# NVlabs/FoundationPose

Measured on AMD Instinct MI355X. Metric: pose-hypotheses/sec (raster+refine+score), 252 hyp x 160x160 @ 640x480 RGB-D, higher is better.
Workload: dtype f16

## Files before the change

### foundationpose_amd/csrc/linear_ln.hip

```cpp
#include <hip/hip_fp16.h>
#include <stdlib.h>
#include <string.h>
#include <type_traits>
#include "igemm_common.h"
#include "rowops_ln.h"

#ifdef FP_PROFILE_BUILD
__device__ unsigned long long ll_dbg[8];
extern "C" int fp_dbg_linear_ln(unsigned long long* out, int reset) {
  if (reset) { unsigned long long z[8] = {0, 0, 0, 0, 0, 0, ~0ull, 0}; return (int)hipMemcpyToSymbol(HIP_SYMBOL(ll_dbg), z, sizeof(z)); }
  return (int)hipMemcpyFromSymbol(out, HIP_SYMBOL(ll_dbg), 8 * sizeof(unsigned long long));
}
#define LL_CLK(t) const unsigned long long t = wall_clock64()
#else
#define LL_CLK(t)
#endif

namespace {

constexpr int LL_BM = 128, LL_BN = 512, LL_K = 512, LL_NW = 8, LL_THREADS = LL_NW * 64, LL_BK = 32;
constexpr int LL_NK = LL_K / LL_BK;
constexpr int LL_KK = LL_BK / 16;
constexpr int LL_TM = LL_BM / 32;
constexpr int LL_ROWB = LL_BK * 2;
constexpr int LL_A_BLOCK = LL_BM * LL_ROWB;
constexpr int LL_E_BYTES = LL_BM * LL_BN * 2;
constexpr int LL_LDS = LL_E_BYTES + LL_BN * 4;
constexpr int LL_ROWS_PER_WAVE = LL_BM / LL_NW, LL_R = 4;
constexpr int LL_LA = 6, LL_LW = 2;
static_assert(LL_NK * LL_A_BLOCK == LL_E_BYTES && LL_LDS <= 160 * 1024, "tile does not fit the 160 KiB LDS");
static_assert(LL_LA > LL_LW && LL_NK > LL_LA, "request order: A block j + LA - LW goes out just before weight fragment j");

struct LinearLnParams {
  const _Float16* X;
  const _Float16* Wp;
  const float* bias;
  const float* x32;
  const _Float16* tok16;
  const float* pe;
  int S;
  const float* gamma;
  const float* beta;
  float eps;
  float* y32;
  _Float16* y16;
  int M;
  int ldx;
  float* part;
  const _Float16* W2p;
  const float* bias2;
  const _Float16* W1p;
  const float* bias1;
};

__global__ __launch_bounds__(256) void k_pack_w512(const _Float16* __restrict__ W, _Float16* __restrict__ out, int K) {
  const int o = blockIdx.x * 256 + threadIdx.x;
  const int lane = o & 63, i = (o >> 6) & 1, rest = o >> 7, nq = K / 16;
  const int q = rest % nq, w = rest / nq;
  if (w >= LL_BN / 64) return;
  const half8 v = *reinterpret_cast<const half8*>(W + (size_t)(64 * w + 32 * i + (lane & 31)) * K + 16 * q + 8 * (lane >> 5));
  *reinterpret_cast<half8*>(out + (size_t)o * 8) = v;
}

__device__ __forceinline__ int ll_swz(int row) { return (row >> 2) & 3; }

__device__ __forceinline__ void ll_dma16(const __amdgpu_buffer_rsrc_t& rs, void* lds, int voff, int soff) {
  __builtin_amdgcn_raw_ptr_buffer_load_lds(rs, (__attribute__((address_space(3))) void*)lds, 16, voff, soff, 0, 0);
}

__device__ __forceinline__ void ll_wait_vm(int n) {
  switch (n) {
    case 0: asm volatile("s_waitcnt vmcnt(0)" ::: "memory"); break;
    case 1: asm volatile("s_waitcnt vmcnt(1)" ::: "memory"); break;
    case 2: asm volatile("s_waitcnt vmcnt(2)" ::: "memory"); break;
    case 4: asm volatile("s_waitcnt vmcnt(4)" ::: "memory"); break;
    case 5: asm volatile("s_waitcnt vmcnt(5)" ::: "memory"); break;
    case 6: asm volatile("s_waitcnt vmcnt(6)" ::: "memory"); break;
    case 8: asm volatile("s_waitcnt vmcnt(8)" ::: "memory"); break;
    case 9: asm volatile("s_waitcnt vmcnt(9)" ::: "memory"); break;
    case 10: asm volatile("s_waitcnt vmcnt(10)" ::: "memory"); break;
    default: asm volatile("s_waitcnt vmcnt(0)" ::: "memory"); break;
  }
}

__device__ __forceinline__ constexpr int ll_after_w(int k1) {
  int n = 0;
  for (int j = k1 + 1; j < LL_NK && j <= k1 - 1 + LL_LW; ++j) n += 4;
  for (int j = k1 + 1; j <= k1 - 1 + LL_LW; ++j) n += (j + LL_LA - LL_LW < LL_NK) ? 1 : 0;
  return n;
}

template <bool MEAN, bool FFN, bool TAIL = false>
__global__ __launch_bounds__(LL_THREADS, 1) void k_rows512(LinearLnParams p) {
  static_assert(!TAIL || (MEAN && FFN), "the tail form ends in the FFN + token-mean form");
  extern __shared__ __attribute__((aligned(16))) unsigned char smem[];
  const int tid = threadIdx.x, lane = tid & 63;
  const int wid = __builtin_amdgcn_readfirstlane(tid >> 6);
  float* bias_lds = reinterpret_cast<float*>(smem + LL_E_BYTES);
  const int m0 = blockIdx.x * LL_BM;
  LL_CLK(t_start);

  if (wid < 2) {
    float* dst = bias_lds + wid * 256;
    if (p.bias) {
      const __amdgpu_buffer_rsrc_t rs = __builtin_amdgcn_make_buffer_rsrc(const_cast<float*>(p.bias), 0, LL_BN * 4, 0x00020000);
      ll_dma16(rs, dst, lane * 16, wid * 1024);
    } else {
      *reinterpret_cast<float4_*>(dst + lane * 4) = float4_{0.f, 0.f, 0.f, 0.f};
    }
  }

  unsigned aoff32;
  {
    const int row = wid * 16 + lane / 4;
    const int c = (lane % 4) ^ ll_swz(row);
    int m = m0 + row;
    m = m < p.M ? m : p.M - 1;
    aoff32 = (unsigned)(((size_t)m * p.ldx + c * 8) * 2);
  }
  const __amdgpu_buffer_rsrc_t rsA = __builtin_amdgcn_make_buffer_rsrc(const_cast<_Float16*>(p.X), 0, 0x7FFFFFFF, 0x00020000);
  auto request_a = [&](int ks) { ll_dma16(rsA, smem + ks * LL_A_BLOCK + wid * 1024, (int)aoff32, ks * (LL_BK * 2)); };
  half8 wr[LL_LW + 1][LL_KK][2];
  auto request_w = [&](const _Float16* wp, int ks, int slot) {
    const _Float16* src = wp + ((size_t)wid * (LL_K / 16) + ks * LL_KK) * 1024 + lane * 8;
#pragma unroll
    for (int kk = 0; kk < LL_KK; ++kk)
#pragma unroll
      for (int i = 0; i < 2; ++i) wr[slot][kk][i] = *reinterpret_cast<const half8*>(src + (kk * 2 + i) * 512);
  };

  float16_ acc[2][LL_TM];
#pragma unroll
  for (int i = 0; i < 2; ++i)
#pragma unroll
    for (int j = 0; j < LL_TM; ++j)
#pragma unroll
      for (int e = 0; e < 16; ++e) acc[i][j][e] = 0.f;

  const int frow = lane & 31, fhalf = lane >> 5;
  const unsigned char* a_ptr[2][LL_KK];
#pragma unroll
  for (int kk = 0; kk < LL_KK; ++kk) {
    a_ptr[0][kk] = smem + frow * LL_ROWB + (((2 * kk + fhalf) ^ ll_swz(frow)) << 4);
    a_ptr[1][kk] = a_ptr[0][kk] + 8 * LL_A_BLOCK;
  }
  half8 fa[2][LL_TM];
  auto read_a = [&](int ks, int kk, int slot) {
#pragma unroll
    for (int t = 0; t < LL_TM; ++t)
      fa[slot][t] = *reinterpret_cast<const half8*>(a_ptr[ks >> 3][kk] + (ks & 7) * LL_A_BLOCK + t * 32 * LL_ROWB);
  };
  auto mfma_group = [&](int wslot, int kk, int aslot) {
#pragma unroll
    for (int i = 0; i < 2; ++i)
#pragma unroll
      for (int j = 0; j < LL_TM; ++j)
        acc[i][j] = __builtin_amdgcn_mfma_f32_32x32x16_f16(wr[wslot][kk][i], fa[aslot][j], acc[i][j], 0, 0, 0);
  };

#pragma unroll
  for (int j = 0; j < LL_LA - LL_LW; ++j) request_a(j);
#pragma unroll
  for (int j = 0; j < LL_LW; ++j) { request_a(j + LL_LA - LL_LW); request_w(p.Wp, j, j); }
  ll_wait_vm(ll_after_w(0));
  __builtin_amdgcn_s_barrier();
  read_a(0, 0, 0);
#pragma unroll
  for (int ks = 0; ks < LL_NK; ++ks) {
    if (ks + LL_LA < LL_NK) request_a(ks + LL_LA);
    if (ks + LL_LW < LL_NK) request_w(p.Wp, ks + LL_LW, (ks + LL_LW) % (LL_LW + 1));
    read_a(ks, 1, 1);
    __builtin_amdgcn_sched_barrier(0);
    mfma_group(ks % (LL_LW + 1), 0, 0);
    __builtin_amdgcn_sched_barrier(0);
    if (ks + 1 < LL_NK) {
      ll_wait_vm(ll_after_w(ks + 1));
      __builtin_amdgcn_s_barrier();
      read_a(ks + 1, 0, 0);
    }
    __builtin_amdgcn_sched_barrier(0);
    mfma_group(ks % (LL_LW + 1), 1, 1);
    __builtin_amdgcn_sched_barrier(0);
  }
  __syncthreads();
  LL_CLK(t_loop1);
  half8 tk[LL_R];
  float rs[LL_R][8];
  auto tile_row = [&](int k) { return MEAN ? wid * LL_ROWS_PER_WAVE + k : wid + LL_NW * k; };
  auto request_resid = [&](int t0, const float* x32) {
#pragma unroll
    for (int u = 0; u < LL_R; ++u) {
      const int m = m0 + tile_row(t0 + u);
      const int mc = m < p.M ? m : p.M - 1;
      if (x32) {
        load8f(x32 + (size_t)mc * 512 + lane * 8, rs[u]);
      } else {
        tk[u] = *reinterpret_cast<const half8*>(p.tok16 + (size_t)mc * 512 + lane * 8);
        load8f(p.pe + (size_t)((unsigned)mc % (unsigned)p.S) * 512 + lane * 8, rs[u]);
      }
    }
  };
  constexpr bool EARLY_RESID = !FFN;
  const float* const resid32 = TAIL ? p.y32 : p.x32;
  if constexpr (EARLY_RESID) request_resid(0, resid32);

  unsigned char* E = smem;
  LL_CLK(t_pre);
  unsigned erow_off = (unsigned)(frow * (2 * LL_BN));
  int esw = frow & 15, efh = fhalf;
  auto read_e = [&](int q, int slot) {
    const unsigned char* erow = E + erow_off;
#pragma unroll
    for (int j = 0; j < LL_TM; ++j)
      fa[slot][j] = *reinterpret_cast<const half8*>(erow + j * 32 * (2 * LL_BN) + (((2 * q + efh) ^ esw) << 4));
  };
  auto zero_acc = [&]() {
#pragma unroll
    for (int i = 0; i < 2; ++i)
#pragma unroll
      for (int j = 0; j < LL_TM; ++j)
#pragma unroll
        for (int e = 0; e < 16; ++e) acc[i][j][e] = 0.f;
  };
  auto product_from_e = [&](const _Float16* wp) {
    asm volatile("" : "+v"(erow_off), "+v"(esw), "+v"(efh));
#pragma unroll
    for (int j = 0; j < LL_LW; ++j) request_w(wp, j, j);
    read_e(0, 0);
#pragma unroll
    for (int ks = 0; ks < LL_NK; ++ks) {
      if (ks + LL_LW < LL_NK) request_w(wp, ks + LL_LW, (ks + LL_LW) % (LL_LW + 1));
      read_e(2 * ks + 1, 1);
      __builtin_amdgcn_sched_barrier(0);
      mfma_group(ks % (LL_LW + 1), 0, 0);
      __builtin_amdgcn_sched_barrier(0);
      if (ks + 1 < LL_NK) read_e(2 * ks + 2, 0);
      __builtin_amdgcn_sched_barrier(0);
      mfma_group(ks % (LL_LW + 1), 1, 1);
      __builtin_amdgcn_sched_barrier(0);
    }
  };
  auto park = [&](auto relu_c) {
    constexpr bool RELU = decltype(relu_c)::value;
    int lane_p = lane;
    asm volatile("" : "+v"(lane_p));
#pragma unroll
    for (int i = 0; i < 2; ++i) {
#pragma unroll
      for (int g = 0; g < 4; ++g) {
        const int nl = wid * 64 + i * 32 + 8 * g + 4 * (lane_p >> 5);
        const float4_ bv = *reinterpret_cast<const float4_*>(bias_lds + nl);
#pragma unroll
        for (int j = 0; j < LL_TM; ++j) {
          const int ml = j * 32 + (lane_p & 31);
          half4 v;
#pragma unroll
          for (int e = 0; e < 4; ++e) v[e] = (_Float16)(acc[i][j][g * 4 + e] + bv[e]);
          if constexpr (RELU) v = __builtin_elementwise_max(v, half4{0, 0, 0, 0});
          const int chunk = (nl >> 3) ^ (ml & 15);
          *reinterpret_cast<half4*>(E + ml * (2 * LL_BN) + (chunk << 4) + ((nl & 4) << 1)) = v;
        }
      }
    }
  };
  auto load_bias = [&](const float* b) {
    if (wid < 2) {
      float* dst = bias_lds + wid * 256;
      if (b) {
        const __amdgpu_buffer_rsrc_t rs_ = __builtin_amdgcn_make_buffer_rsrc(const_cast<float*>(b), 0, LL_BN * 4, 0x00020000);
        ll_dma16(rs_, dst, lane * 16, wid * 1024);
      } else {
        *reinterpret_cast<float4_*>(dst + lane * 4) = float4_{0.f, 0.f, 0.f, 0.f};
      }
    }
  };
  if constexpr (TAIL) {
    request_resid(0, nullptr);
    park(std::false_type{});
    __syncthreads();
    {
      float gm1[8], bt1[8];
      load8f(p.gamma + lane * 8, gm1);
      load8f(p.beta + lane * 8, bt1);
#pragma unroll 1
      for (int t0 = 0; t0 < LL_ROWS_PER_WAVE; t0 += LL_R) {
        float f[LL_R][8];
#pragma unroll
        for (int u = 0; u < LL_R; ++u) {
          const int r = tile_row(t0 + u);
          const half8 b = *reinterpret_cast<const half8*>(E + r * (2 * LL_BN) + ((lane ^ (r & 15)) << 4));
#pragma unroll
          for (int e = 0; e < 8; ++e) {
            f[u][e] = (float)tk[u][e] + rs[u][e];
            f[u][e] += (float)b[e];
          }
        }
        if (t0 + LL_R < LL_ROWS_PER_WAVE) request_resid(t0 + LL_R, nullptr);
        ln_rows<LL_R>(p.eps, f);
#pragma unroll
        for (int u = 0; u < LL_R; ++u) {
          const int r = tile_row(t0 + u);
          const int m = m0 + r;
          half8 h;
#pragma unroll
          for (int e = 0; e < 8; ++e) { f[u][e] = fmaf(f[u][e], gm1[e], bt1[e]); h[e] = (_Float16)f[u][e]; }
          if (m < p.M) store8f(p.y32 + (size_t)m * 512 + lane * 8, f[u]);
          *reinterpret_cast<half8*>(E + r * (2 * LL_BN) + ((lane ^ (r & 15)) << 4)) = h;
        }
      }
    }
    __syncthreads();
    load_bias(p.bias1);
    zero_acc();
    product_from_e(p.W1p);
    asm volatile("s_waitcnt vmcnt(0)" ::: "memory");
    __syncthreads();
  }
  if constexpr (FFN) {
    park(std::true_type{});
    __syncthreads();
    load_bias(p.bias2);
    zero_acc();
    product_from_e(p.W2p);
    asm volatile("s_waitcnt vmcnt(0)" ::: "memory");
    __syncthreads();
  }
  LL_CLK(t_loop2);
  park(std::false_type{});
  __syncthreads();
  LL_CLK(t_park);
  if constexpr (!EARLY_RESID) request_resid(0, resid32);

  float gm[8], bt[8];
  if constexpr (!MEAN) {
    load8f(p.gamma + lane * 8, gm);
    load8f(p.beta + lane * 8, bt);
  }
  float csum[8];
#pragma unroll
  for (int e = 0; e < 8; ++e) csum[e] = 0.f;
#pragma unroll 1
  for (int t0 = 0; t0 < LL_ROWS_PER_WAVE; t0 += LL_R) {
    float f[LL_R][8];
#pragma unroll
    for (int u = 0; u < LL_R; ++u) {
      const int r = tile_row(t0 + u);
      const half8 b = *reinterpret_cast<const half8*>(E + r * (2 * LL_BN) + ((lane ^ (r & 15)) << 4));
#pragma unroll
      for (int e = 0; e < 8; ++e) {
        f[u][e] = resid32 ? rs[u][e] : (float)tk[u][e] + rs[u][e];
        f[u][e] += (float)b[e];
      }
    }
    if (t0 + LL_R < LL_ROWS_PER_WAVE) request_resid(t0 + LL_R, resid32);
    ln_rows<LL_R>(p.eps, f);
    if constexpr (MEAN) {
#pragma unroll
      for (int u = 0; u < LL_R; ++u) {
        const int m = m0 + tile_row(t0 + u);
        if (m >= p.M) continue;
#pragma unroll
        for (int e = 0; e < 8; ++e) csum[e] += f[u][e];
      }
      continue;
    }
#pragma unroll
    for (int u = 0; u < LL_R; ++u) {
      const int m = m0 + tile_row(t0 + u);
      if (m >= p.M) continue;
      half8 h;
#pragma unroll
      for (int e = 0; e < 8; ++e) { f[u][e] = fmaf(f[u][e], gm[e], bt[e]); h[e] = (_Float16)f[u][e]; }
      if (p.y32) store8f(p.y32 + (size_t)m * 512 + lane * 8, f[u]);
      if (p.y16) *reinterpret_cast<half8*>(p.y16 + (size_t)m * 512 + lane * 8) = h;
    }
  }
  if constexpr (MEAN) {
    static_assert(!MEAN || LL_ROWS_PER_WAVE == 16, "a wave's chunk is 16 rows: groups are multiples of 16 rows");
    const int mrow = m0 + wid * LL_ROWS_PER_WAVE;
    if (mrow < p.M) store8f(p.part + (size_t)(mrow / LL_ROWS_PER_WAVE) * 512 + lane * 8, csum);
  }
#ifdef FP_PROFILE_BUILD
  asm volatile("s_waitcnt vmcnt(0)" ::: "memory");
  LL_CLK(t_end);
  if (tid == 0) {
    atomicAdd(&ll_dbg[0], t_loop1 - t_start); atomicAdd(&ll_dbg[1], t_loop2 - t_pre); atomicAdd(&ll_dbg[2], t_park - t_loop2);
    atomicAdd(&ll_dbg[3], t_end - t_park); atomicAdd(&ll_dbg[4], 1ull); atomicMin(&ll_dbg[6], t_start); atomicMax(&ll_dbg[7], t_end);
  }
#endif
}

struct Linear512Params {
  const _Float16* X;
  const _Float16* Wp;
  const float* bias;
  _Float16* Y;
  int M, N, relu;
};
constexpr int L5_XBUF = 32 * 64;
constexpr int L5_BIAS_OFF = LL_E_BYTES + LL_NW * L5_XBUF;
constexpr int L5_MAX_N = 3072;
constexpr int l5_lds(int N) { return L5_BIAS_OFF + N * 4; }
static_assert(l5_lds(L5_MAX_N) <= 160 * 1024, "tile does not fit the 160 KiB LDS");

__global__ __launch_bounds__(LL_THREADS, 1) void k_linear512(Linear512Params p) {
  extern __shared__ __attribute__((aligned(16))) unsigned char smem[];
  const int tid = threadIdx.x, lane = tid & 63;
  const int wid = __builtin_amdgcn_readfirstlane(tid >> 6);
  float* bias_lds = reinterpret_cast<float*>(smem + L5_BIAS_OFF);
  unsigned char* xbuf = smem + LL_E_BYTES + wid * L5_XBUF;
  const int m0 = blockIdx.x * LL_BM;
  const int nblk = p.N / LL_BN;

  for (int q = wid; q < p.N / 256; q += LL_NW) {
    float* dst = bias_lds + q * 256;
    if (p.bias) {
      const __amdgpu_buffer_rsrc_t rs = __builtin_amdgcn_make_buffer_rsrc(const_cast<float*>(p.bias), 0, p.N * 4, 0x00020000);
      ll_dma16(rs, dst, lane * 16, q * 1024);
    } else {
      *reinterpret_cast<float4_*>(dst + lane * 4) = float4_{0.f, 0.f, 0.f, 0.f};
    }
  }
  unsigned aoff32;
  {
    const int row = wid * 16 + lane / 4;
    const int c = (lane % 4) ^ ll_swz(row);
    int m = m0 + row;
    m = m < p.M ? m : p.M - 1;
    aoff32 = (unsigned)(((size_t)m * LL_K + c * 8) * 2);
  }
  const __amdgpu_buffer_rsrc_t rsA = __builtin_amdgcn_make_buffer_rsrc(const_cast<_Float16*>(p.X), 0, 0x7FFFFFFF, 0x00020000);
  auto request_a = [&](int ks) { ll_dma16(rsA, smem + ks * LL_A_BLOCK + wid * 1024, (int)aoff32, ks * (LL_BK * 2)); };
  half8 wr[LL_LW + 1][LL_KK][2];
  auto request_w = [&](const _Float16* wp, int ks, int slot) {
    const _Float16* src = wp + ((size_t)wid * (LL_K / 16) + ks * LL_KK) * 1024 + lane * 8;
#pragma unroll
    for (int kk = 0; kk < LL_KK; ++kk)
#pragma unroll
      for (int i = 0; i < 2; ++i) wr[slot][kk][i] = *reinterpret_cast<const half8*>(src + (kk * 2 + i) * 512);
  };
  float16_ acc[2][LL_TM];
  const int frow = lane & 31, fhalf = lane >> 5;
  const unsigned char* a_ptr[2][LL_KK];
#pragma unroll
  for (int kk = 0; kk < LL_KK; ++kk) {
    a_ptr[0][kk] = smem + frow * LL_ROWB + (((2 * kk + fhalf) ^ ll_swz(frow)) << 4);
    a_ptr[1][kk] = a_ptr[0][kk] + 8 * LL_A_BLOCK;
  }
  half8 fa[2][LL_TM];
  auto read_a = [&](int ks, int kk, int slot) {
#pragma unroll
    for (int t = 0; t < LL_TM; ++t)
      fa[slot][t] = *reinterpret_cast<const half8*>(a_ptr[ks >> 3][kk] + (ks & 7) * LL_A_BLOCK + t * 32 * LL_ROWB);
  };
  auto mfma_group = [&](int wslot, int kk, int aslot) {
#pragma unroll
    for (int i = 0; i < 2; ++i)
#pragma unroll
      for (int j = 0; j < LL_TM; ++j)
        acc[i][j] = __builtin_amdgcn_mfma_f32_32x32x16_f16(wr[wslot][kk][i], fa[aslot][j], acc[i][j], 0, 0, 0);
  };
  auto zero_acc = [&]() {
#pragma unroll
    for (int i = 0; i < 2; ++i)
#pragma unroll
      for (int j = 0; j < LL_TM; ++j)
#pragma unroll
        for (int e = 0; e < 16; ++e) acc[i][j][e] = 0.f;
  };
  auto store_block = [&](int nb) {
    const half4 zero4 = {0, 0, 0, 0};
#pragma unroll
    for (int i = 0; i < 2; ++i) {
      const int nl = nb * LL_BN + wid * 64 + i * 32;
#pragma unroll
      for (int j = 0; j < LL_TM; ++j) {
#pragma unroll
        for (int g = 0; g < 4; ++g) {
          const float4_ bv = *reinterpret_cast<const float4_*>(bias_lds + nl + 8 * g + 4 * fhalf);
          half4 v;
#pragma unroll
          for (int e = 0; e < 4; ++e) v[e] = (_Float16)(acc[i][j][g * 4 + e] + bv[e]);
          if (p.relu) v = __builtin_elementwise_max(v, zero4);
          *reinterpret_cast<half4*>(xbuf + frow * 64 + ((g ^ ll_swz(frow)) << 4) + 8 * fhalf) = v;
        }
        __builtin_amdgcn_s_waitcnt(0xc07f);
        __builtin_amdgcn_wave_barrier();
#pragma unroll
        for (int h = 0; h < 2; ++h) {
          const int r = h * 16 + (lane >> 2), c = lane & 3;
          const half8 o = *reinterpret_cast<const half8*>(xbuf + r * 64 + ((c ^ ll_swz(r)) << 4));
          const int m = m0 + j * 32 + r;
          if (m < p.M) *reinterpret_cast<half8*>(p.Y + (size_t)m * p.N + nl + c * 8) = o;
        }
        __builtin_amdgcn_s_waitcnt(0xc07f);
        __builtin_amdgcn_wave_barrier();
      }
    }
  };

  zero_acc();
#pragma unroll
  for (int j = 0; j < LL_LA - LL_LW; ++j) request_a(j);
#pragma unroll
  for (int j = 0; j < LL_LW; ++j) { request_a(j + LL_LA - LL_LW); request_w(p.Wp, j, j); }
  ll_wait_vm(ll_after_w(0));
  __builtin_amdgcn_s_barrier();
  read_a(0, 0, 0);
#pragma unroll
  for (int ks = 0; ks < LL_NK; ++ks) {
    if (ks + LL_LA < LL_NK) request_a(ks + LL_LA);
    if (ks + LL_LW < LL_NK) request_w(p.Wp, ks + LL_LW, (ks + LL_LW) % (LL_LW + 1));
    read_a(ks, 1, 1);
    __builtin_amdgcn_sched_barrier(0);
    mfma_group(ks % (LL_LW + 1), 0, 0);
    __builtin_amdgcn_sched_barrier(0);
    if (ks + 1 < LL_NK) {
      ll_wait_vm(ll_after_w(ks + 1));
      __builtin_amdgcn_s_barrier();
      read_a(ks + 1, 0, 0);
    }
    __builtin_amdgcn_sched_barrier(0);
    mfma_group(ks % (LL_LW + 1), 1, 1);
    __builtin_amdgcn_sched_barrier(0);
  }
  if (nblk > 1) {
#pragma unroll
    for (int j = 0; j < LL_LW; ++j) request_w(p.Wp + (size_t)LL_BN * LL_K, j, j);
  }
  store_block(0);
#pragma unroll 1
  for (int nb = 1; nb < nblk; ++nb) {
    const _Float16* wp = p.Wp + (size_t)nb * LL_BN * LL_K;
    zero_acc();
    read_a(0, 0, 0);
#pragma unroll
    for (int ks = 0; ks < LL_NK; ++ks) {
      if (ks + LL_LW < LL_NK) request_w(wp, ks + LL_LW, (ks + LL_LW) % (LL_LW + 1));
      read_a(ks, 1, 1);
      __builtin_amdgcn_sched_barrier(0);
      mfma_group(ks % (LL_LW + 1), 0, 0);
      __builtin_amdgcn_sched_barrier(0);
      if (ks + 1 < LL_NK) read_a(ks + 1, 0, 0);
      __builtin_amdgcn_sched_barrier(0);
      mfma_group(ks % (LL_LW + 1), 1, 1);
      __builtin_amdgcn_sched_barrier(0);
    }
    if (nb + 1 < nblk) {
#pragma unroll
      for (int j = 0; j < LL_LW; ++j) request_w(wp + (size_t)LL_BN * LL_K, j, j);
    }
    store_block(nb);
  }
}

__global__ __launch_bounds__(512) void k_ln_mean_finish(const float* __restrict__ part, const float* __restrict__ gamma,
                                                       const float* __restrict__ beta, float* __restrict__ out, int S) {
  const int g = blockIdx.x, c = threadIdx.x;
  const int nch = S / 16;
  const float* src = part + (size_t)g * nch * 512 + c;
  float a = 0.f;
  for (int k = 0; k < nch; ++k) a += src[(size_t)k * 512];
  a *= 1.0f / (float)S;
  out[(size_t)g * 512 + c] = fmaf(a, gamma[c], beta[c]);
}

}

extern "C" int fp_pack_linear512_f16(const void* w16, void* packed, void* stream) {
  FP_REQUIRE(w16 && packed, "fp_pack_linear512_f16: NULL tensor");
  FP_REQUIRE(w16 != packed, "fp_pack_linear512_f16: cannot pack in place");
  FP_REQUIRE((((size_t)w16 | (size_t)packed) & 15) == 0, "fp_pack_linear512_f16: tensors must be 16-byte aligned");
  hipLaunchKernelGGL(k_pack_w512, dim3(LL_BN * LL_K / 8 / 256), dim3(256), 0, (hipStream_t)stream, (const _Float16*)w16, (_Float16*)packed,
                     LL_K);
  FP_CHECK_LAUNCH("fp_pack_linear512_f16");
  return FP_OK;
}

extern "C" int fp_linear512_f16_fwd(const void* x16, const void* w_packed, const float* bias, void* y16, int M, int N, int relu,
                                    void* stream) {
  FP_REQUIRE(M >= 0, "fp_linear512_f16_fwd: M < 0");
  if (M == 0) return FP_OK;
  FP_REQUIRE(x16 && w_packed && y16, "fp_linear512_f16_fwd: NULL tensor");
  FP_REQUIRE(N >= LL_BN && N % LL_BN == 0 && N <= L5_MAX_N, "fp_linear512_f16_fwd: N=%d must be a multiple of 512, at most %d", N, L5_MAX_N);
  FP_REQUIRE((long long)M * N < (1ll << 31), "fp_linear512_f16_fwd: output exceeds 2^31 elements");
  FP_REQUIRE((((size_t)x16 | (size_t)w_packed | (size_t)bias | (size_t)y16) & 15) == 0, "fp_linear512_f16_fwd: tensors must be 16-byte aligned");
  Linear512Params p;
  p.X = (const _Float16*)x16; p.Wp = (const _Float16*)w_packed; p.bias = bias; p.Y = (_Float16*)y16; p.M = M; p.N = N; p.relu = relu ? 1 : 0;
  const int lds = l5_lds(N);
  FP_SET_MAX_LDS(k_linear512, l5_lds(L5_MAX_N));
  hipLaunchKernelGGL(k_linear512, dim3(fp_cdiv(M, LL_BM)), dim3(LL_THREADS), lds, (hipStream_t)stream, p);
  FP_CHECK_LAUNCH("fp_linear512_f16_fwd");
  return FP_OK;
}

extern "C" int fp_ffn_layernorm_mean_fwd(const void* y16, const void* w1_packed, const float* b1, const void* w2_packed, const float* b2,
                                         const float* x32, const float* gamma, const float* beta, float eps, float* out,
                                         float* workspace, size_t workspace_bytes, int groups, int rows_per_group, void* stream) {
  FP_REQUIRE(groups >= 0, "fp_ffn_layernorm_mean_fwd: groups < 0");
  if (groups == 0) return FP_OK;
  FP_REQUIRE(y16 && w1_packed && w2_packed && x32 && gamma && beta && out && workspace, "fp_ffn_layernorm_mean_fwd: NULL tensor");
  FP_REQUIRE(rows_per_group >= 16 && rows_per_group % 16 == 0,
             "fp_ffn_layernorm_mean_fwd: rows_per_group=%d must be a multiple of 16 (a wave sums 16 consecutive rows, which have to belong to one group)", rows_per_group);
  const long long M = (long long)groups * rows_per_group;
  FP_REQUIRE(M * 512 < (1ll << 30), "fp_ffn_layernorm_mean_fwd: operands exceed 2 GiB");
  FP_REQUIRE((((size_t)y16 | (size_t)w1_packed | (size_t)w2_packed | (size_t)b1 | (size_t)b2 | (size_t)x32 | (size_t)gamma | (size_t)beta) & 15) == 0,
             "fp_ffn_layernorm_mean_fwd: tensors must be 16-byte aligned");
  const int tiles = fp_cdiv((int)M, LL_BM);
  FP_REQUIRE(workspace_bytes >= (size_t)(M / 16) * 512 * sizeof(float), "fp_ffn_layernorm_mean_fwd: workspace too small");
  LinearLnParams p;
  p.X = (const _Float16*)y16; p.Wp = (const _Float16*)w1_packed; p.bias = b1; p.x32 = x32; p.tok16 = nullptr; p.pe = nullptr;
  p.S = rows_per_group; p.gamma = gamma; p.beta = beta; p.eps = eps; p.y32 = nullptr; p.y16 = nullptr; p.M = (int)M; p.ldx = LL_K;
  p.part = workspace; p.W2p = (const _Float16*)w2_packed; p.bias2 = b2; p.W1p = nullptr; p.bias1 = nullptr;
  FP_SET_MAX_LDS((k_rows512<true, true>), LL_LDS);
  hipLaunchKernelGGL((k_rows512<true, true>), dim3(tiles), dim3(LL_THREADS), LL_LDS, (hipStream_t)stream, p);
  hipLaunchKernelGGL(k_ln_mean_finish, dim3(groups), dim3(512), 0, (hipStream_t)stream, (const float*)workspace, gamma, beta, out,
                     rows_per_group);
  FP_CHECK_LAUNCH("fp_ffn_layernorm_mean_fwd");
  return FP_OK;
}

extern "C" size_t fp_encoder_tail_workspace_bytes(int groups, int rows_per_group) {
  if (groups <= 0 || rows_per_group <= 0) return 0;
  const size_t M = (size_t)groups * rows_per_group;
  return M * 512 * sizeof(float) + (M / 16 + 1) * 512 * sizeof(float);
}

extern "C" int fp_encoder_tail_mean_fwd(const void* ctx16, int ldx, const void* wo_packed, const float* bo, const void* tok16, const float* pe,
                                        const float* gamma1, const float* beta1, const void* w1_packed, const float* b1,
                                        const void* w2_packed, const float* b2, const float* gamma2, const float* beta2, float eps,
                                        float* out, void* workspace, size_t workspace_bytes, int groups, int rows_per_group, void* stream) {
  FP_REQUIRE(groups >= 0, "fp_encoder_tail_mean_fwd: groups < 0");
  if (groups == 0) return FP_OK;
  FP_REQUIRE(ctx16 && wo_packed && tok16 && pe && gamma1 && beta1 && w1_packed && w2_packed && gamma2 && beta2 && out && workspace,
             "fp_encoder_tail_mean_fwd: NULL tensor");
  FP_REQUIRE(rows_per_group >= 16 && rows_per_group % 16 == 0,
             "fp_encoder_tail_mean_fwd: rows_per_group=%d must be a multiple of 16 (a wave sums 16 consecutive rows, which have to belong to one group)", rows_per_group);
  if (ldx == 0) ldx = LL_K;
  FP_REQUIRE(ldx >= LL_K && ldx % 8 == 0, "fp_encoder_tail_mean_fwd: ldx=%d must be a multiple of 8 and at least 512", ldx);
  const long long M = (long long)groups * rows_per_group;
  FP_REQUIRE(M * ldx < (1ll << 30), "fp_encoder_tail_mean_fwd: operands exceed 2 GiB");
  FP_REQUIRE((((size_t)ctx16 | (size_t)wo_packed | (size_t)bo | (size_t)tok16 | (size_t)pe | (size_t)gamma1 | (size_t)beta1 | (size_t)w1_packed |
               (size_t)b1 | (size_t)w2_packed | (size_t)b2 | (size_t)gamma2 | (size_t)beta2 | (size_t)workspace) & 15) == 0,
             "fp_encoder_tail_mean_fwd: tensors must be 16-byte aligned");
  const size_t need = fp_encoder_tail_workspace_bytes(groups, rows_per_group);
  if (workspace_bytes < need) {
    fp_set_error("fp_encoder_tail_mean_fwd: workspace too small (%zu < %zu bytes, see fp_encoder_tail_workspace_bytes)", workspace_bytes, need);
    return FP_ERR_WORKSPACE;
  }
  LinearLnParams p;
  p.X = (const _Float16*)ctx16; p.ldx = ldx; p.Wp = (const _Float16*)wo_packed; p.bias = bo; p.x32 = nullptr; p.tok16 = (const _Float16*)tok16;
  p.pe = pe; p.S = rows_per_group; p.gamma = gamma1; p.beta = beta1; p.eps = eps; p.y16 = nullptr; p.M = (int)M;
  p.y32 = (float*)workspace;
  p.part = (float*)workspace + (size_t)M * 512;
  p.W1p = (const _Float16*)w1_packed; p.bias1 = b1; p.W2p = (const _Float16*)w2_packed; p.bias2 = b2;
  FP_SET_MAX_LDS((k_rows512<true, true, true>), LL_LDS);
  hipLaunchKernelGGL((k_rows512<true, true, true>), dim3(fp_cdiv((int)M, LL_BM)), dim3(LL_THREADS), LL_LDS, (hipStream_t)stream, p);
  hipLaunchKernelGGL(k_ln_mean_finish, dim3(groups), dim3(512), 0, (hipStream_t)stream, (const float*)p.part, gamma2, beta2, out, rows_per_group);
  FP_CHECK_LAUNCH("fp_encoder_tail_mean_fwd");
  return FP_OK;
}

extern "C" int fp_linear_layernorm_fwd(const void* x16, const void* w16_packed, const float* bias, const float* x32, const void* tok16,
                                       const float* pe, int S, const float* gamma, const float* beta, float eps, float* y32,
                                       void* y16, int M, int K, int D, int ldx, void* stream) {
  FP_REQUIRE(M >= 0, "fp_linear_layernorm_fwd: M < 0");
  if (M == 0) return FP_OK;
  FP_REQUIRE(x16 && w16_packed && gamma && beta && (y32 || y16), "fp_linear_layernorm_fwd: NULL tensor");
  FP_REQUIRE((x32 != nullptr) != (tok16 != nullptr), "fp_linear_layernorm_fwd: give the residual as x32 OR as tok16 (+ pe)");
  FP_REQUIRE(x32 || (pe && S > 0), "fp_linear_layernorm_fwd: tok16 needs the positional table and its period");
  FP_REQUIRE(D == 512 && K == 512, "fp_linear_layernorm_fwd: K=%d D=%d unsupported (d_model of both networks is 512; the A tile of 128 rows x K lives in LDS whole)", K, D);
  if (ldx == 0) ldx = K;
  FP_REQUIRE(ldx >= K && ldx % 8 == 0, "fp_linear_layernorm_fwd: ldx=%d must be a multiple of 8 and at least K", ldx);
  FP_REQUIRE((long long)M * ldx < (1ll << 30), "fp_linear_layernorm_fwd: operands exceed 2 GiB");
  FP_REQUIRE((((size_t)x16 | (size_t)w16_packed | (size_t)bias | (size_t)x32 | (size_t)tok16 | (size_t)pe | (size_t)gamma | (size_t)beta |
               (size_t)y32 | (size_t)y16) & 15) == 0, "fp_linear_layernorm_fwd: tensors must be 16-byte aligned");
  LinearLnParams p;
  p.X = (const _Float16*)x16; p.Wp = (const _Float16*)w16_packed; p.bias = bias; p.x32 = x32; p.tok16 = (const _Float16*)tok16; p.pe = pe;
  p.S = S; p.gamma = gamma; p.beta = beta; p.eps = eps; p.y32 = y32; p.y16 = (_Float16*)y16; p.M = M; p.ldx = ldx; p.part = nullptr; p.W2p = nullptr; p.bias2 = nullptr; p.W1p = nullptr; p.bias1 = nullptr;
  FP_SET_MAX_LDS((k_rows512<false, false>), LL_LDS);
  hipLaunchKernelGGL((k_rows512<false, false>), dim3(fp_cdiv(M, LL_BM)), dim3(LL_THREADS), LL_LDS, (hipStream_t)stream, p);
  FP_CHECK_LAUNCH("fp_linear_layernorm_fwd");
  return FP_OK;
}
```

Before: 7185.

## Make linear512 kernel persistent over balanced (row-tile, N-block) work items

The 512-K linear kernel now launches at most one workgroup per CU. Each workgroup walks a contiguous range of (row tile, N block) items instead of owning one row tile across all N blocks. When a workgroup crosses into the next row tile, it prefetches the next tile's A and W while storing the previous result. Weight loads move to buffer loads with a byte-offset resource. The intent is to balance load and remove the tail effect when the number of row tiles does not divide well across CUs, at the cost of more complex control flow and a per-device CU-count lookup on the host.

```diff
diff --git a/foundationpose_amd/csrc/linear512_items.h b/foundationpose_amd/csrc/linear512_items.h
--- /dev/null
+++ b/foundationpose_amd/csrc/linear512_items.h
@@ -0,0 +1,18 @@
+#pragma once
+#ifdef __HIPCC__
+#define L5_HD __host__ __device__
+#else
+#define L5_HD
+#endif
+
+struct L5Range {
+  int first, end;
+};
+
+L5_HD inline int l5_grid(int items, int cus) { return items < cus ? items : cus; }
+
+L5_HD inline L5Range l5_range(int items, int wgs, int g) {
+  const int q = items / wgs, r = items % wgs;
+  const int first = g * q + (g < r ? g : r);
+  return L5Range{first, first + q + (g < r ? 1 : 0)};
+}
diff --git a/foundationpose_amd/csrc/linear_ln.hip b/foundationpose_amd/csrc/linear_ln.hip
--- a/foundationpose_amd/csrc/linear_ln.hip
+++ b/foundationpose_amd/csrc/linear_ln.hip
@@ -3,6 +3,7 @@
 #include <string.h>
 #include <type_traits>
 #include "igemm_common.h"
+#include "linear512_items.h"
 #include "rowops_ln.h"
 
 #ifdef FP_PROFILE_BUILD
@@ -409,8 +410,10 @@
   const int wid = __builtin_amdgcn_readfirstlane(tid >> 6);
   float* bias_lds = reinterpret_cast<float*>(smem + L5_BIAS_OFF);
   unsigned char* xbuf = smem + LL_E_BYTES + wid * L5_XBUF;
-  const int m0 = blockIdx.x * LL_BM;
   const int nblk = p.N / LL_BN;
+  const L5Range range = l5_range((p.M + LL_BM - 1) / LL_BM * nblk, gridDim.x, blockIdx.x);
+  int item = range.first;
+  int nb = item % nblk, m0 = item / nblk * LL_BM;
 
   for (int q = wid; q < p.N / 256; q += LL_NW) {
     float* dst = bias_lds + q * 256;
@@ -421,23 +424,32 @@
       *reinterpret_cast<float4_*>(dst + lane * 4) = float4_{0.f, 0.f, 0.f, 0.f};
     }
   }
+  auto lane_id = []() {
+    int l;
+    asm volatile("v_mbcnt_lo_u32_b32 %0, -1, 0\n\tv_mbcnt_hi_u32_b32 %0, -1, %0" : "=v"(l));
+    return l;
+  };
   unsigned aoff32;
-  {
+  auto set_tile = [&](int mt) {
+    const int lane = lane_id();
     const int row = wid * 16 + lane / 4;
     const int c = (lane % 4) ^ ll_swz(row);
-    int m = m0 + row;
+    int m = mt + row;
     m = m < p.M ? m : p.M - 1;
     aoff32 = (unsigned)(((size_t)m * LL_K + c * 8) * 2);
-  }
+  };
+  set_tile(m0);
   const __amdgpu_buffer_rsrc_t rsA = __builtin_amdgcn_make_buffer_rsrc(const_cast<_Float16*>(p.X), 0, 0x7FFFFFFF, 0x00020000);
   auto request_a = [&](int ks) { ll_dma16(rsA, smem + ks * LL_A_BLOCK + wid * 1024, (int)aoff32, ks * (LL_BK * 2)); };
+  const __amdgpu_buffer_rsrc_t rsW = __builtin_amdgcn_make_buffer_rsrc(const_cast<_Float16*>(p.Wp), 0, p.N * LL_K * 2, 0x00020000);
   half8 wr[LL_LW + 1][LL_KK][2];
-  auto request_w = [&](const _Float16* wp, int ks, int slot) {
-    const _Float16* src = wp + ((size_t)wid * (LL_K / 16) + ks * LL_KK) * 1024 + lane * 8;
+  auto request_w = [&](int nb, int ks, int slot) {
+    const int soff = nb * (LL_BN * LL_K * 2) + (wid * (LL_K / 16) + ks * LL_KK) * 2048;
 #pragma unroll
     for (int kk = 0; kk < LL_KK; ++kk)
 #pragma unroll
-      for (int i = 0; i < 2; ++i) wr[slot][kk][i] = *reinterpret_cast<const half8*>(src + (kk * 2 + i) * 512);
+      for (int i = 0; i < 2; ++i)
+        wr[slot][kk][i] = __builtin_bit_cast(half8, __builtin_amdgcn_raw_buffer_load_b128(rsW, lane * 16 + (kk * 2 + i) * 1024, soff, 0));
   };
   float16_ acc[2][LL_TM];
   const int frow = lane & 31, fhalf = lane >> 5;
@@ -468,7 +480,8 @@
 #pragma unroll
         for (int e = 0; e < 16; ++e) acc[i][j][e] = 0.f;
   };
-  auto store_block = [&](int nb) {
+  auto store_block = [&](int nb, int mt) {
+    const int lane = lane_id(), frow = lane & 31, fhalf = lane >> 5;
     const half4 zero4 = {0, 0, 0, 0};
 #pragma unroll
     for (int i = 0; i < 2; ++i) {
@@ -490,7 +503,7 @@
         for (int h = 0; h < 2; ++h) {
           const int r = h * 16 + (lane >> 2), c = lane & 3;
           const half8 o = *reinterpret_cast<const half8*>(xbuf + r * 64 + ((c ^ ll_swz(r)) << 4));
-          const int m = m0 + j * 32 + r;
+          const int m = mt + j * 32 + r;
           if (m < p.M) *reinterpret_cast<half8*>(p.Y + (size_t)m * p.N + nl + c * 8) = o;
         }
         __builtin_amdgcn_s_waitcnt(0xc07f);
@@ -499,59 +512,73 @@
     }
   };
 
-  zero_acc();
-#pragma unroll
-  for (int j = 0; j < LL_LA - LL_LW; ++j) request_a(j);
-#pragma unroll
-  for (int j = 0; j < LL_LW; ++j) { request_a(j + LL_LA - LL_LW); request_w(p.Wp, j, j); }
-  ll_wait_vm(ll_after_w(0));
-  __builtin_amdgcn_s_barrier();
-  read_a(0, 0, 0);
-#pragma unroll
-  for (int ks = 0; ks < LL_NK; ++ks) {
-    if (ks + LL_LA < LL_NK) request_a(ks + LL_LA);
-    if (ks + LL_LW < LL_NK) request_w(p.Wp, ks + LL_LW, (ks + LL_LW) % (LL_LW + 1));
-    read_a(ks, 1, 1);
-    __builtin_amdgcn_sched_barrier(0);
-    mfma_group(ks % (LL_LW + 1), 0, 0);
-    __builtin_amdgcn_sched_barrier(0);
-    if (ks + 1 < LL_NK) {
-      ll_wait_vm(ll_after_w(ks + 1));
-      __builtin_amdgcn_s_barrier();
-      read_a(ks + 1, 0, 0);
-    }
-    __builtin_amdgcn_sched_barrier(0);
-    mfma_group(ks % (LL_LW + 1), 1, 1);
-    __builtin_amdgcn_sched_barrier(0);
-  }
-  if (nblk > 1) {
-#pragma unroll
-    for (int j = 0; j < LL_LW; ++j) request_w(p.Wp + (size_t)LL_BN * LL_K, j, j);
-  }
-  store_block(0);
+  auto request_first = [&](int nb) {
+#pragma unroll
+    for (int j = 0; j < LL_LA - LL_LW; ++j) request_a(j);
+#pragma unroll
+    for (int j = 0; j < LL_LW; ++j) { request_a(j + LL_LA - LL_LW); request_w(nb, j, j); }
+  };
+  auto first_block = [&](int nb) {
+    ll_wait_vm(ll_after_w(0));
+    __builtin_amdgcn_s_barrier();
+    read_a(0, 0, 0);
+#pragma unroll
+    for (int ks = 0; ks < LL_NK; ++ks) {
+      if (ks + LL_LA < LL_NK) request_a(ks + LL_LA);
+      if (ks + LL_LW < LL_NK) request_w(nb, ks + LL_LW, (ks + LL_LW) % (LL_LW + 1));
+      read_a(ks, 1, 1);
+      __builtin_amdgcn_sched_barrier(0);
+      mfma_group(ks % (LL_LW + 1), 0, 0);
+      __builtin_amdgcn_sched_barrier(0);
+      if (ks + 1 < LL_NK) {
+        ll_wait_vm(ll_after_w(ks + 1));
+        __builtin_amdgcn_s_barrier();
+        read_a(ks + 1, 0, 0);
+      }
+      __builtin_amdgcn_sched_barrier(0);
+      mfma_group(ks % (LL_LW + 1), 1, 1);
+      __builtin_amdgcn_sched_barrier(0);
+    }
+  };
+  auto next_block = [&](int nb) {
+    read_a(0, 0, 0);
+#pragma unroll
+    for (int ks = 0; ks < LL_NK; ++ks) {
+      if (ks + LL_LW < LL_NK) request_w(nb, ks + LL_LW, (ks + LL_LW) % (LL_LW + 1));
+      read_a(ks, 1, 1);
+      __builtin_amdgcn_sched_barrier(0);
+      mfma_group(ks % (LL_LW + 1), 0, 0);
+      __builtin_amdgcn_sched_barrier(0);
+      if (ks + 1 < LL_NK) read_a(ks + 1, 0, 0);
+      __builtin_amdgcn_sched_barrier(0);
+      mfma_group(ks % (LL_LW + 1), 1, 1);
+      __builtin_amdgcn_sched_barrier(0);
+    }
+  };
+
+  request_first(nb);
 #pragma unroll 1
-  for (int nb = 1; nb < nblk; ++nb) {
-    const _Float16* wp = p.Wp + (size_t)nb * LL_BN * LL_K;
+  for (;;) {
     zero_acc();
-    read_a(0, 0, 0);
-#pragma unroll
-    for (int ks = 0; ks < LL_NK; ++ks) {
-      if (ks + LL_LW < LL_NK) request_w(wp, ks + LL_LW, (ks + LL_LW) % (LL_LW + 1));
-      read_a(ks, 1, 1);
-      __builtin_amdgcn_sched_barrier(0);
-      mfma_group(ks % (LL_LW + 1), 0, 0);
-      __builtin_amdgcn_sched_barrier(0);
-      if (ks + 1 < LL_NK) read_a(ks + 1, 0, 0);
-      __builtin_amdgcn_sched_barrier(0);
-      mfma_group(ks % (LL_LW + 1), 1, 1);
-      __builtin_amdgcn_sched_barrier(0);
-    }
-    if (nb + 1 < nblk) {
-#pragma unroll
-      for (int j = 0; j < LL_LW; ++j) request_w(wp + (size_t)LL_BN * LL_K, j, j);
-    }
-    store_block(nb);
-  }
+    first_block(nb);
+#pragma unroll 1
+    while (++item < range.end && nb + 1 < nblk) {
+      ++nb;
+#pragma unroll
+      for (int j = 0; j < LL_LW; ++j) request_w(nb, j, j);
+      store_block(nb - 1, m0);
+      zero_acc();
+      next_block(nb);
+    }
+    if (item == range.end) break;
+    set_tile(m0 + LL_BM);
+    __builtin_amdgcn_s_barrier();
+    request_first(0);
+    store_block(nb, m0);
+    nb = 0;
+    m0 += LL_BM;
+  }
+  store_block(nb, m0);
 }
 
 __global__ __launch_bounds__(512) void k_ln_mean_finish(const float* __restrict__ part, const float* __restrict__ gamma,
@@ -587,9 +614,21 @@
   FP_REQUIRE((((size_t)x16 | (size_t)w_packed | (size_t)bias | (size_t)y16) & 15) == 0, "fp_linear512_f16_fwd: tensors must be 16-byte aligned");
   Linear512Params p;
   p.X = (const _Float16*)x16; p.Wp = (const _Float16*)w_packed; p.bias = bias; p.Y = (_Float16*)y16; p.M = M; p.N = N; p.relu = relu ? 1 : 0;
+  static std::atomic<int> n_cu[64];
+  int dev = 0;
+  (void)hipGetDevice(&dev);
+  int cus = dev >= 0 && dev < 64 ? n_cu[dev].load(std::memory_order_relaxed) : 0;
+  if (cus == 0) {
+    const hipError_t e = hipDeviceGetAttribute(&cus, hipDeviceAttributeMultiprocessorCount, dev);
+    if (e != hipSuccess || cus <= 0) {
+      fp_set_error("fp_linear512_f16_fwd: cannot read the CU count of device %d: %s", dev, hipGetErrorString(e));
+      return FP_ERR_LAUNCH;
+    }
+    if (dev >= 0 && dev < 64) n_cu[dev].store(cus, std::memory_order_relaxed);
+  }
   const int lds = l5_lds(N);
   FP_SET_MAX_LDS(k_linear512, l5_lds(L5_MAX_N));
-  hipLaunchKernelGGL(k_linear512, dim3(fp_cdiv(M, LL_BM)), dim3(LL_THREADS), lds, (hipStream_t)stream, p);
+  hipLaunchKernelGGL(k_linear512, dim3(l5_grid(fp_cdiv(M, LL_BM) * (N / LL_BN), cus)), dim3(LL_THREADS), lds, (hipStream_t)stream, p);
   FP_CHECK_LAUNCH("fp_linear512_f16_fwd");
   return FP_OK;
 }
```

Result: no change. 7184, median of 6 (-0.0%).
